# nanoporetech/tombo

Hardware: AMD Instinct MI355X
Metric: resquiggle reads/s (10 kb DNA, bw=500) (higher is better)
Workload: dtype f64

## Files before the change

include/tombo_amd.h:

```cpp
#ifndef TOMBO_AMD_H
#define TOMBO_AMD_H
#include <stdint.h>

#ifdef __cplusplus
extern "C" {
#endif

enum {
    TBA_OK = 0,
    TBA_TOO_MUCH_SIGNAL = 1,
    TBA_FEWER_CPTS = 2,
    TBA_READ_TOO_SHORT_START = 3,
    TBA_MAP_TOO_SHORT_START = 4,
    TBA_POOR_START = 5,
    TBA_INVALID_START_PATH = 6,
    TBA_OPEN_PORE = 7,
    TBA_STARTS_TOO_FAR = 8,
    TBA_MASK_TOO_FEW = 9,
    TBA_ADAPT_BEYOND = 10,
    TBA_BEYOND_BANDWIDTH = 11,
    TBA_DISCORDANT = 12,
    TBA_NOT_ENOUGH_DEL_SIGNAL = 13,
    TBA_TOO_MANY_DELS = 14,
    TBA_INVALID_SEG = 15,
// ... 101 lines not shown
enum {
    TBA_GET_VALID_CPTS = 1,
    TBA_GET_N_CPTS = 2,
    TBA_GET_EVENT_MEANS = 3,
    TBA_GET_SEG_NORM = 4,
    TBA_GET_SEG_SV = 5,
    TBA_GET_START = 6,
    TBA_GET_BAND_STARTS = 7,
    TBA_GET_READ_TB = 8,
    TBA_GET_DP_SEGS = 9,
    TBA_GET_THEIL_SEN = 10,
    TBA_GET_PATH = 11,
    TBA_GET_LAST_ROW = 12,
    TBA_GET_DP_READ_START = 13,
    TBA_GET_KERNEL_MS = 14,
    TBA_GET_REF_MEANS = 15,
    TBA_GET_REF_SDS = 16,
    TBA_GET_SEGS = 17,
    TBA_GET_STATUS = 18,
    TBA_GET_START_FAIL = 19,
    TBA_GET_STALL_INTS = 20,
    TBA_GET_N_STALL = 21,
    TBA_GET_STALL_OFF = 22,
    TBA_GET_SAMP_IND = 23,
    TBA_GET_TB_PARALLEL = 24,
    TBA_GET_ED_FUSED = 25,
    TBA_GET_ED_TAKEN_POS = 26,
    TBA_GET_ED_N_TAKEN = 27,
    TBA_GET_DP_WORKGROUP = 28,
    TBA_GET_ED_FORM = 29,
    TBA_GET_TB_FORM = 30,
    TBA_GET_TB_VERIFY_FAIL = 31,
    TBA_GET_DP_FORM = 32,
    TBA_GET_DEBUG_COUNTERS = 99
};
enum {
    TBA_ED_FORM_NONE = 0,
    TBA_ED_FORM_WG_SCAN_PEAKS = 1,
    TBA_ED_FORM_DETECT_PICK = 2,
    TBA_ED_FORM_SCORES_PEAKS = 3,
    TBA_ED_FORM_DETECT_TT_PICK = 4,
    TBA_ED_FORM_TTEST_PEAKS = 5
};
enum {
    TBA_TB_FORM_NONE = 0,
    TBA_TB_FORM_LANE = 1,
    TBA_TB_FORM_LONG = 2,
    TBA_TB_FORM_PAR16 = 16,
    TBA_TB_FORM_PAR64 = 64
};
enum {
    TBA_DP_FORM_NONE = 0,
    TBA_DP_FORM_K_DP = 1,
    TBA_DP_FORM_K_DP8_LOWREG = 2,
    TBA_DP_FORM_MULTI = 3,
    TBA_DP_FORM_WIDE = 4
};
enum {
    TBA_DP_START_NONE = 0,
    TBA_DP_START_FIRST_TRY = 1,
    TBA_DP_START_RETRY_WG = 2,
    TBA_DP_START_RETRY_K_DP = 3
};
int tba_batch_get(tba_engine *e, int what, void *out, int64_t out_bytes);
enum {
    TBA_STAGE_SEGMENT = 0,
    TBA_STAGE_EVENT_MEANS = 1,
    TBA_STAGE_REF_LEVELS = 2,
    TBA_STAGE_START = 3,
    TBA_STAGE_ASSIGN = 4,
    TBA_STAGE_SKIP = 5,
    TBA_STAGE_RESCALE = 6
};
enum {
    TBA_PUT_VALID_CPTS = 1,
// ... 206 lines not shown
```

tombo_amd/_native.py:

```python
import os
import ctypes as C
import subprocess
from collections import namedtuple

import numpy as np

from ._default_parameters import MAX_POINTS_FOR_THEIL_SEN, SIG_MATCH_THRESH

_HERE = os.path.dirname(os.path.abspath(__file__))
LIB_PATH = os.environ.get('TBA_LIB_PATH') or os.path.join(_HERE, 'libtombo_amd.so')
CSRC = os.path.join(_HERE, 'csrc')
i64, f64, i32 = C.c_int64, C.c_double, C.c_int32

HIPCC_FLAGS = ['--offload-arch=gfx950', '-O3', '-std=c++17', '-ffp-contract=off', '-fPIC',
               '-shared']


INJECT_LIB_PATH = os.path.join(_HERE, 'libtombo_amd_inject.so')
INJECT_FLAGS = ['-DTBA_TB_INJECT=5']


def build(force=False):
    tree_lib = os.path.join(_HERE, 'libtombo_amd.so')
    srcs = [os.path.join(CSRC, f) for f in sorted(os.listdir(CSRC))] + \
# ... 35 lines not shown
                ('device_subsample', i64), ('subsample_seed', C.c_uint64), ('subsample_first_read', i64),
                ('del_fix_window', i64), ('max_del_fix_window', i64), ('extra_sig_factor', f64)]


class ReadResult(C.Structure):
    _fields_ = [('status', i32), ('norm_params_changed', i32),
                ('read_start_rel_to_raw', i64), ('norm_len', i64),
                ('shift', f64), ('scale', f64), ('lower_lim', f64), ('upper_lim', f64),
                ('sig_match_score', f64)]


class SynthParams(C.Structure):
    _fields_ = [('mean_dwell', i64), ('min_dwell', i64), ('n_lead', i64), ('n_trail', i64),
                ('scale', f64), ('offset', f64), ('noise_sd', f64), ('dac_per_pa', f64), ('dac_offset', f64),
                ('reverse', i32), ('pad', i32)]


RESULT_DTYPE = np.dtype([
    ('status', np.int32), ('norm_params_changed', np.int32),
    ('read_start_rel_to_raw', np.int64), ('norm_len', np.int64),
    ('shift', np.float64), ('scale', np.float64), ('lower_lim', np.float64),
    ('upper_lim', np.float64), ('sig_match_score', np.float64)])
assert RESULT_DTYPE.itemsize == C.sizeof(ReadResult) == 64

RAW_F64, RAW_F32, RAW_I16 = 0, 1, 2
RAW_DTYPES = {np.dtype(np.float64): RAW_F64, np.dtype(np.float32): RAW_F32,
              np.dtype(np.int16): RAW_I16}


GET_VALID_CPTS, GET_N_CPTS, GET_EVENT_MEANS, GET_SEG_NORM, GET_SEG_SV, GET_START, \
    GET_BAND_STARTS, GET_READ_TB, GET_DP_SEGS, GET_THEIL_SEN, GET_PATH, GET_LAST_ROW, \
    GET_DP_READ_START, GET_KERNEL_MS, GET_REF_MEANS, GET_REF_SDS, GET_SEGS, GET_STATUS, GET_START_FAIL, \
    GET_STALL_INTS, GET_N_STALL, GET_STALL_OFF, GET_SAMP_IND, GET_TB_PARALLEL, GET_ED_FUSED, GET_ED_TAKEN_POS, GET_ED_N_TAKEN, \
    GET_DP_WORKGROUP, GET_ED_FORM, GET_TB_FORM, GET_TB_VERIFY_FAIL, GET_DP_FORM = range(1, 33)
ED_FORM_NONE, ED_FORM_WG_SCAN_PEAKS, ED_FORM_DETECT_PICK, ED_FORM_SCORES_PEAKS, ED_FORM_DETECT_TT_PICK, \
    ED_FORM_TTEST_PEAKS = range(6)
TB_FORM_NONE, TB_FORM_LANE, TB_FORM_LONG, TB_FORM_PAR16, TB_FORM_PAR64 = 0, 1, 2, 16, 64
DP_FORM_NONE, DP_FORM_K_DP, DP_FORM_K_DP8_LOWREG, DP_FORM_MULTI, DP_FORM_WIDE = range(5)
DP_START_NONE, DP_START_FIRST_TRY, DP_START_RETRY_WG, DP_START_RETRY_K_DP = range(4)
GET_DEBUG_COUNTERS = 99
STAGE_SEGMENT, STAGE_EVENT_MEANS, STAGE_REF_LEVELS, STAGE_START, STAGE_ASSIGN, STAGE_SKIP, \
    STAGE_RESCALE = range(7)
PUT_VALID_CPTS, PUT_EVENT_MEANS, PUT_NORM, PUT_REF_MEANS, PUT_REF_SDS, PUT_DP_SEGS, \
    PUT_START_STATE = range(1, 8)
MAX_BAND = 3072
ABI_VERSION = 12
STAGE_NAMES = ["normalize", "cumsum", "scores", "peaks", "event_means", "ref_levels",
               "start_dp", "start_tb", "prep", "main_dp", "main_tb", "skip_resolve", "theil_sen",
               "rescale_score", "stalls", "total"]

_GET_SHAPES = {
    GET_N_CPTS: (np.int64, ('n',)), GET_DP_READ_START: (np.int64, ('n',)),
    GET_SEG_SV: (np.float64, ('n', 4)), GET_START: (np.float64, ('n', 4)),
    GET_THEIL_SEN: (np.float64, ('n', 4)), GET_PATH: (np.int32, ('n', 4)), GET_DP_FORM: (np.int32, ('n', 4)),
    GET_LAST_ROW: (np.float64, ('n', MAX_BAND)), GET_KERNEL_MS: (np.float32, (32,)),
    GET_DEBUG_COUNTERS: (np.int64, ('n', 8)),
    GET_VALID_CPTS: (np.int64, ('ev',)), GET_EVENT_MEANS: (np.float64, ('ev',)),
    GET_SEG_NORM: (np.float64, ('raw',)),
    GET_BAND_STARTS: (np.int64, ('ref',)), GET_REF_MEANS: (np.float64, ('ref',)), GET_REF_SDS: (np.float64, ('ref',)),
    GET_READ_TB: (np.int64, ('seg',)), GET_DP_SEGS: (np.int64, ('seg',)), GET_SEGS: (np.int64, ('seg',)),
    GET_STATUS: (np.int32, ('n',)), GET_START_FAIL: (np.int32, ('n',)),
    GET_N_STALL: (np.int64, ('n',)), GET_STALL_OFF: (np.int64, ('n',)),
    GET_SAMP_IND: (np.int64, ('n', MAX_POINTS_FOR_THEIL_SEN)),
    GET_TB_PARALLEL: (np.int32, ('n',)), GET_ED_FUSED: (np.int32, ('n',)), GET_DP_WORKGROUP: (np.int32, ('n',)),
    GET_ED_FORM: (np.int32, ('n',)), GET_TB_FORM: (np.int32, ('n',)), GET_TB_VERIFY_FAIL: (np.int32, ('n',)),
    GET_ED_TAKEN_POS: (np.int32, ('raw_x2',)), GET_ED_N_TAKEN: (np.int64, ('n',)),
}

class _Ptr(object):
    _CTYPES = (C.c_int.__mro__[-2], type(C.byref(C.c_int())))

    def __init__(self, dtype, const):
        self.dtype, self.const = np.dtype(dtype), const

    def from_param(self, a):
        if a is None or isinstance(a, self._CTYPES):
            return a
        if isinstance(a, np.ndarray):
            if a.dtype == self.dtype and a.flags.c_contiguous and (self.const or a.flags.writeable):
                return C.c_void_p(a.ctypes.data)
        elif isinstance(a, DeviceArray) and a.dtype == self.dtype:
            return C.c_void_p(a.ptr)
        raise TypeError('expected None, a C-contiguous %s%s array or a ctypes object, got %s' % (
            '' if self.const else 'writeable ', self.dtype, getattr(a, 'dtype', type(a).__name__)))


def _prototypes():
    n, q, u, d, v = C.c_int, i64, C.c_uint64, f64, C.c_void_p
    D, Q, I, B = (_Ptr(t, False) for t in (np.float64, np.int64, np.int32, np.uint8))
    cD, cQ, cI, cB, cS = (_Ptr(t, True) for t in (np.float64, np.int64, np.int32, np.uint8, np.int8))
    P, O, R, SP = (C.POINTER(t) for t in (Params, Opts, ReadResult, SynthParams))
    pileup = [q, cQ, cQ, cS, cQ, q, cQ, cS]
    site_outs = [D, Q, Q, Q, D, Q, Q]
    fwd_pass = [v, D, Q, q, q, Q, cD, q, cD, cD, d, d, d, q, d, n, d]
    return {
        'tba_engine_create': (n, [n, v]),
        'tba_engine_destroy': (None, [v]),
        'tba_last_error': (C.c_char_p, []),
# ... 1369 lines not shown
```

tombo_amd/csrc/k_segment.h:

```cpp
#pragma once
#include "k_select.h"

template <class RT> struct raw_is_int { static constexpr bool value = false; };
template <> struct raw_is_int<int16_t> { static constexpr bool value = true; };
#define NORM_WINDOW_MIN 16384

template <class RT>
__global__ __launch_bounds__(SEL_NT, 4) void k_normalize(ReadState *rs, const DevParams *dp,
    const RT *raw, double *norm, const double *sv_in, int mode, int write_norm)
{
    __shared__ BucketSmem sm;
    ReadState &r = rs[blockIdx.x];
    if (r.status != TBA_OK) return;
    const int tid = threadIdx.x;
    const StampClock<phase_on(PH_NORMALIZE)> stamps(r.dbg);
    const i64 n = r.n_raw;
    const RawSamples<RT> x{raw + r.raw_off};
    double *y = norm + r.raw_off;
    const tba_opts &o = dp->o;
    double shift, scale, lo = 0, hi = 0;
    double xlo = 0, xhi = 0, mn = 0, mx = 0;
    bool have_lims = false, have_dev = false;
    double dlo = 0, dhi = 0;
    if (r.sv_flags & 1) {
        shift = sv_in[4 * blockIdx.x + 0];
        scale = sv_in[4 * blockIdx.x + 1];
        if (r.sv_flags & 2) { have_lims = true; lo = sv_in[4 * blockIdx.x + 2]; hi = sv_in[4 * blockIdx.x + 3]; }
    } else if (mode == 1 && !o.has_const_scale && o.use_rna_event_scale) {
        shift = r.shift; scale = r.scale; have_lims = true; lo = r.lower; hi = r.upper;
    } else {
        double samp[WS_PER];
        double smn = INFINITY, smx = -INFINITY;
#pragma unroll
        for (int q = 0; q < WS_PER; q++) {
            const i64 si = (n * (i64)(q * SEL_NT + tid)) / (SEL_NT * WS_PER);
            samp[q] = x[si];
            smn = samp[q] < smn ? samp[q] : smn; smx = samp[q] > smx ? samp[q] : smx;
        }
        for (int mm = 32; mm >= 1; mm >>= 1) {
            double a = shfl_xor_f64(smn, mm), b2 = shfl_xor_f64(smx, mm);
            smn = a < smn ? a : smn; smx = b2 > smx ? b2 : smx;
        }
        if ((tid & 63) == 0) { sm.redd[2 * (tid >> 6)] = smn; sm.redd[2 * (tid >> 6) + 1] = smx; }
        __syncthreads();
        smn = sm.redd[0]; smx = sm.redd[1];
        for (int w = 1; w < SEL_NT / 64; w++) {
            smn = sm.redd[2 * w] < smn ? sm.redd[2 * w] : smn;
            smx = sm.redd[2 * w + 1] > smx ? sm.redd[2 * w + 1] : smx;
        }
        __syncthreads();
        double span = smx - smn;
        span = span > 0 ? span : 1.0;
        mn = smn - span; mx = smx + span;
        stamps.stamp(0);
        bool have_med = false;
        if constexpr (raw_is_int<RT>::value) {
            if (n >= 4096 && block_int_medians(x, n, (int)smn, (int)smx, &sm, &xlo, &xhi, &dlo, &dhi)) {
                shift = (n & 1) ? xlo : (xlo + xhi) / 2.0;
                have_med = true;
                if (!o.has_const_scale) { scale = (n & 1) ? dlo : (dlo + dhi) / 2.0; have_dev = true; }
            }
            __syncthreads();
        }
        const bool thresh = o.has_outlier_thresh && !(mode == 1 && !o.has_const_scale);
        double med = 0, mad = 0;
#pragma nounroll
        for (int what = 0; what < 3; what++) {
            if (what == 0 && have_med) continue;
            if (what == 1) {
                if (o.has_const_scale) { scale = o.const_scale; continue; }
                if (have_dev) continue;
            }
            if (what == 2) {
                if (!thresh) break;
                const double ylo = (xlo - shift) / scale, yhi = (xhi - shift) / scale;
                med = (n & 1) ? ylo : (ylo + yhi) / 2.0;
                if (have_dev && med == 0.0 && scale > 0) {
                    const double m_lo = dlo / scale, m_hi = dhi / scale;
                    mad = (n & 1) ? m_lo : (m_lo + m_hi) / 2.0;
                    break;
                }
            }
            auto of = [&](double xv) {
                return what == 0 ? xv : (what == 1 ? fabs(xv - shift) : fabs((xv - shift) / scale - med));
            };
            auto val = [&](i64 i) { return of(x[i]); };
            double a_lo = 0, a_hi = 0, res = 0;
            bool done = false;
            if (!raw_is_int<RT>::value && n >= NORM_WINDOW_MIN) {
                double ds[WS_PER];
#pragma unroll
                for (int q = 0; q < WS_PER; q++) ds[q] = of(samp[q]);
                done = block_median_window<2>(x, of, n, ds, y, n, &sm, &a_lo, &a_hi);
                if (done) res = (n & 1) ? a_lo : (a_lo + a_hi) / 2.0;
                __syncthreads();
            }
// ... 771 lines not shown
```

tombo_amd/csrc/k_select.h:

```cpp
#pragma once
#include "tba_common.h"

template <int U, class Load, class Body>
__device__ __forceinline__ void block_stream(i64 n, Load load, Body body)
{
    const i64 tid = threadIdx.x, nt = blockDim.x;
    i64 base = 0;
    for (; base + (i64)U * nt <= n; base += (i64)U * nt) {
        decltype(load((i64)0)) v[U];
#pragma unroll
        for (int u = 0; u < U; u++) v[u] = load(base + (i64)u * nt + tid);
#pragma unroll
        for (int u = 0; u < U; u++) body(base + (i64)u * nt + tid, v[u]);
    }
    for (i64 i = base + tid; i < n; i += nt) body(i, load(i));
}

template <int U, class Sig, class Body>
__device__ __forceinline__ void block_stream2(i64 n, Sig x, Body body)
{
    const i64 tid = threadIdx.x, nt = blockDim.x, np = n >> 1;
    i64 base = 0;
    for (; base + (i64)U * nt <= np; base += (i64)U * nt) {
        double a[U], b[U];
// ... 655 lines not shown
            const i64 a = (shift2 - e) / 2 - base, b2 = (shift2 + e) / 2 - base;
            i64 cnt = 0;
            if (a >= 0 && a < BS_NB) cnt += sm->hist[a];
            if (e != 0 && b2 >= 0 && b2 < BS_NB) cnt += sm->hist[b2];
            c += cnt; loc[q] = c;
        }
        i64 inc = c;
        for (int d = 1; d < 64; d <<= 1) {
            i64 t = shfl_i64(inc, (tid & 63) - d < 0 ? 0 : (tid & 63) - d);
            if ((tid & 63) >= d) inc += t;
        }
        __syncthreads();
        if ((tid & 63) == 63) sm->rad.red[tid >> 6] = (u64)inc;
        __syncthreads();
        i64 off = 0;
        for (int w = 0; w < (tid >> 6); w++) off += (i64)sm->rad.red[w];
        const i64 exc = off + inc - c;
        i64 tot = 0;
        for (int w = 0; w < SEL_NT / 64; w++) tot += (i64)sm->rad.red[w];
        if (tid == 0) s_okk = (tot == n - below - above) && k_hi < tot;
#pragma unroll
        for (int q = 0; q < per; q++) {
            const i64 lo_c = exc + (q ? loc[q - 1] : 0), hi_c = exc + loc[q];
            const i64 e = par + 2 * (i64)(tid * per + q);
            if (lo_c <= k_lo && k_lo < hi_c) s_k[2] = e;
            if (lo_c <= k_hi && k_hi < hi_c) s_k[3] = e;
        }
    }
    __syncthreads();
    if (!s_okk) return false;
    if (below > 0 && (shift2 - s_k[3]) / 2 < (i64)base) return false;
    if (above > 0 && (shift2 + s_k[3]) / 2 > (i64)base + BS_NB - 1) return false;
    *dlo = (double)s_k[2] / 2.0; *dhi = (double)s_k[3] / 2.0;
    return true;
}


__device__ __forceinline__ double seq_sum_lds(const double *p, int j0, int j1, double s = 0)
{
    int j = j0;
    for (; j + 8 <= j1; j += 8) {
        double t[8];
#pragma unroll
        for (int u = 0; u < 8; u++) t[u] = p[j + u];
#pragma unroll
        for (int u = 0; u < 8; u++) s += t[u];
    }
    for (; j < j1; j++) s += p[j];
    return s;
}

template <int SEGW_CAP, class Sig, class F, class Pre, class Emit>
__device__ __forceinline__ void wave_segment_sums(Sig x,
    const i64 *__restrict__ seg, i64 n_segs, i64 first_group, i64 group_stride, double *lds,
    double *out, F f, Pre pre, Emit emit, double mean_len)
{
    constexpr int NP = (SEGW_CAP + 127) / 128;
    const int lane = threadIdx.x & 63;
    int gs = 64;
    while (gs > 4 && (double)gs * mean_len * 1.3 > (double)SEGW_CAP) gs >>= 1;
    i64 g = first_group;
    if (g * gs >= n_segs) return;
    struct Raw { i64 a, hi; };
    auto load_raw = [&](i64 gg) {
        const i64 i = gg * gs + lane;
        const bool ok = lane < gs && i < n_segs;
// ... 165 lines not shown
```

tombo_amd/csrc/tba_common.h:

```cpp
#pragma once
#include <hip/hip_runtime.h>
#include <stdint.h>
#include "../../include/tombo_amd.h"

typedef int64_t i64;
typedef uint64_t u64;
typedef int32_t i32;
typedef uint32_t u32;

#define MASK_BASES 50
#define MASK_FILL_Z_SCORE (-15.0)
#define DEL_FIX_WINDOW 2
#define MAX_DEL_FIX_WINDOW 10
#define EXTRA_SIG_FACTOR 1.1
#define SHIFT_CHANGE_THRESH 0.1
#define SCALE_CHANGE_THRESH 0.1
#define MAX_TS_POINTS 1000

#include "tba_phase.h"

enum { PATH_NONE = 0, PATH_ADAPTIVE = 1, PATH_STATIC = 2 };
enum { ST_NONE = 0, ST_TRY = 1, ST_OK = 2, ST_RETRY = 3, ST_STATIC = 4 };

struct ReadState {
    i64 raw_off, n_raw;
    i64 seq_off, seq_len;
    i64 ref_off, B;
    i64 seg_off;
    i64 ev_off, num_events;
    i64 stall_off, n_stall;
    i32 status, path, start_state, sv_flags;
    i32 n_start_calls, changed, pad0;
    i32 is_long;
    double shift, scale, lower, upper;
    i32 has_lims;
    i32 tb_done;
    i32 ed_flag, dp_wg;
    i32 ed_form, tb_form;
    i32 strip_s0;
    i32 bad_seq;
    i32 tb_verify_fail, pad1;
    i64 n_taken;
    double ed_min, ed_max;
    i64 n_cpts, n_ev;
    double start_res[4];
    i64 mapped_start; double epb;
    i64 clip, offset, W, n_static, moves_off, top_pos;
    i64 read_start, norm_len, dp_read_start;
    i64 n_win, skip_off;
    double ts[4]; double score;
    i64 dbg[8];
};

struct DevParams {
    tba_params p;
    tba_opts o;
    i64 kmer_width, central_pos;
    double fill_masked;
    i32 dp_wg_mode, pad;
};

typedef double f64x2_u __attribute__((ext_vector_type(2), aligned(8)));
typedef float f32x2_u __attribute__((ext_vector_type(2), aligned(4)));
typedef short i16x2_u __attribute__((ext_vector_type(2), aligned(2)));
__device__ __forceinline__ void ld2(const double *p, double &a, double &b)
{
    const f64x2_u v = *(const f64x2_u *)p;
    a = v.x; b = v.y;
}
__device__ __forceinline__ void st2(double *p, double a, double b)
{
    f64x2_u v;
    v.x = a; v.y = b;
    *(f64x2_u *)p = v;
// ... 221 lines not shown
```

tombo_amd/csrc/tba_engine.hip:

```cpp
#include <atomic>
#include "tba_common.h"
#include "k_select.h"
#include "k_segment.h"
#include "k_detect.h"
#include "k_prep_raw.h"
#include "k_dp.h"
#include "k_tb_par.h"
#include "k_dp_multi.h"
#include "k_long.h"
#include "k_dp_wg.h"
#include "k_tail.h"
#include "k_cabi.h"
#include "k_synth.h"
#include "k_group.h"
#include "k_site.h"
#include "k_kde.h"
#include "k_tracks.h"
#include "k_kmer_est.h"
#include "k_roc.h"
#include "k_pdist.h"
#include "k_plot.h"

#include <algorithm>
#include <array>
// ... 542 lines not shown
    c.side = !side_off && first == TBA_STAGE_SEGMENT && last == TBA_STAGE_RESCALE && e->side_mode != 0 &&
             (e->side_mode == 1 || (e->device < TBA_MAX_DEVICES &&
              std::max(e->n_sharing, g_live_engines[e->device].load()) <= max_engines));
    e->last_side = c.side;
    if (c.side && !e->stream2) HIP_TRY(hipStreamCreate(&e->stream2));
    const hipStream_t s2 = c.s2 = c.side ? e->stream2 : s;
    if (c.side) {
        HIP_TRY(hipEventRecord(e->ev_fork, s));
        HIP_TRY(hipStreamWaitEvent(s2, e->ev_fork, 0));
    }
    HIP_TRY(hipEventRecord(e->ev_st0, s2));
    if (first == TBA_STAGE_SEGMENT && c.O.detect_stalls) {
        const unsigned gq = c.gx(e->z.max_raw / 8 + 1);
        if (c.rdt == TBA_RAW_I16 && c.O.stall_window_size <= SI_MAXW) {
            (c.O.stall_n_windows == 7 ? k_stall_metric_i16<7> : k_stall_metric_i16<0>)<<<dim3(gq, c.nb), 256, 0, s2>>>(c.rs, c.dp, (int16_t *)c.raw, c.stall_bits);
        } else {
            if (cs_reads_for(c.n) == 20) RAW_DISPATCH(c.rdt, (k_cumsum_scores<20, RT, 1><<<(unsigned)((c.n + 19) / 20), 256, 0, s2>>>(c.rs, c.n, c.dp, (RT *)c.raw, c.stall_csum)));
            else RAW_DISPATCH(c.rdt, (k_cumsum_scores<32, RT, 1><<<(unsigned)((c.n + 31) / 32), 256, 0, s2>>>(c.rs, c.n, c.dp, (RT *)c.raw, c.stall_csum)));
            if (e->n_long > 0) RAW_DISPATCH(c.rdt, (k_cumsum_scores_long<RT, 1><<<(unsigned)e->n_long, 256, 0, s2>>>(c.rs, c.lng, c.dp, (RT *)c.raw, c.stall_csum)));
            (c.O.stall_n_windows == 7 ? k_stall_metric<7> : k_stall_metric<0>)<<<dim3(gq, c.nb), 256, 0, s2>>>(c.rs, c.dp, c.stall_csum, c.stall_bits);
        }
        k_stall_runs<<<dim3(c.gx(e->z.max_raw / 64 + 1), c.nb), 256, 0, s2>>>(c.rs, c.dp, c.stall_bits, c.stall);
        k_stall_merge<<<c.tpr, 64, 0, s2>>>(c.rs, c.n, c.dp, c.stall);
    }
    HIP_TRY(hipEventRecord(e->ev_st1, s2));
    if (c.side) {
        HIP_TRY(hipEventRecord(e->ev_stalls, s2));
        k_ref_levels<<<dim3(c.gB, c.nb), 256, 0, s2>>>(c.rs, c.dp, c.seq, c.kmeans, c.ksds, c.refm, c.refs, 1);
        HIP_TRY(hipEventRecord(e->ev_levels, s2));
    }
    return 0;
}

static int step_normalize(Run &c)
{
    if (!c.rna) RAW_DISPATCH(c.rdt, (k_normalize<RT><<<c.nb, SEL_NT, 0, c.s>>>(c.rs, c.dp, (RT *)c.raw, c.norm, c.sv_in, 0, c.fused_detect && !c.wg_scan ? 2 : 1)));
    return 0;
}
static int step_cumsum(Run &c)
{
    const i64 n = c.n;
    if (c.rna) return 0;
    if (c.wg_scan) {
        k_cumsum_scores_long<double, 0><<<c.nb, 256, 0, c.s>>>(c.rs, c.order, c.dp, c.norm, c.score);
        return 0;
    }
    if (c.fused_detect) {
        RAW_DISPATCH(c.rdt, (k_detect<2, RT><<<(unsigned)((n + DT_READS - 1) / DT_READS), 256, 0, c.s>>>(c.rs, n, c.dp, (RT *)c.raw, c.norm, c.csum, c.score, c.e->z.S_tot)));
        k_pick<<<c.nb, SEL_NT, 0, c.s>>>(c.rs, c.dp, c.csum, c.score, c.cpts, 0);
    }
    if (c.fused_scores) {
        if (cs_reads_for(n) == 20) k_cumsum_scores<20><<<(unsigned)((n + 19) / 20), 256, 0, c.s>>>(c.rs, n, c.dp, c.norm, c.score, c.only_flagged);
        else k_cumsum_scores<32><<<(unsigned)((n + 31) / 32), 256, 0, c.s>>>(c.rs, n, c.dp, c.norm, c.score, c.only_flagged);
        if (c.e->n_long > 0) k_cumsum_scores_long<double, 0><<<(unsigned)c.e->n_long, 256, 0, c.s>>>(c.rs, c.lng, c.dp, c.norm, c.score);
    }
    else k_cumsum<<<c.tpr, 64, 0, c.s>>>(c.rs, n, c.norm, c.csum);
    return 0;
}
static int step_scores(Run &c)
{
    if (!c.rna) {
        if (!c.fused_scores) k_scores_dna<<<dim3(c.gS, c.nb), 256, 0, c.s>>>(c.rs, c.dp, c.csum, c.score);
        return 0;
    }
    if (c.fused_tt) {
        if (c.P.running_stat_width == 12) RAW_DISPATCH(c.rdt, (k_detect_tt<5, 12, RT><<<c.nb, SEL_NT, 0, c.s>>>(c.rs, c.dp, (RT *)c.raw, c.csum, c.score)));
        else RAW_DISPATCH(c.rdt, (k_detect_tt<5, 0, RT><<<c.nb, SEL_NT, 0, c.s>>>(c.rs, c.dp, (RT *)c.raw, c.csum, c.score)));
        k_pick<<<c.nb, SEL_NT, 0, c.s>>>(c.rs, c.dp, c.csum, c.score, c.cpts, 1);
    }
    RAW_DISPATCH(c.rdt, (k_scores_ttest<RT><<<dim3(c.gS, c.nb), 256, 0, c.s>>>(c.rs, c.dp, (RT *)c.raw, c.score, c.only_flagged)));
    return 0;
}
static int step_peaks(Run &c)
{
    launch_peaks(c.P.min_obs_per_base, c.nb, c.s, c.rs, c.dp, c.score, c.state, c.csum, c.cpts, c.rna ? 1 : 0, c.only_flagged,
                 c.rna ? TBA_ED_FORM_TTEST_PEAKS : c.wg_scan ? TBA_ED_FORM_WG_SCAN_PEAKS : TBA_ED_FORM_SCORES_PEAKS);
    if (c.side) HIP_TRY(hipStreamWaitEvent(c.s, c.e->ev_stalls, 0));
    if (c.e->any_stall) k_remove_stalls<<<c.nb, SEL_NT, 0, c.s>>>(c.rs, c.n, c.stall, c.cpts, c.csum);
    if (c.rna) {
        RAW_DISPATCH(c.rdt, (k_event_means<RT, 1280><<<dim3(c.gE, c.nb), 256, 0, c.s>>>(c.rs, c.dp, (RT *)c.raw, c.cpts, c.evm, 1)));
        k_rna_event_scale<<<c.nb, SEL_NT, 0, c.s>>>(c.rs, c.dp, c.evm);
        RAW_DISPATCH(c.rdt, (k_normalize<RT><<<c.nb, SEL_NT, 0, c.s>>>(c.rs, c.dp, (RT *)c.raw, c.norm, c.sv_in, 1, 1)));
    }
    return 0;
}
static int step_event_means(Run &c)
{
    (c.P.mean_obs_per_event >= 10 ? k_event_means<double, 1280> : k_event_means<double>)<<<dim3(c.gE, c.nb), 256, 0, c.s>>>(c.rs, c.dp, c.norm, c.cpts, c.evm, 0);
    return 0;
}
static int step_ref_levels(Run &c)
{
    if (c.side) {
        HIP_TRY(hipStreamWaitEvent(c.s, c.e->ev_levels, 0));
        k_seq_status<<<c.tpr, 64, 0, c.s>>>(c.rs, c.n);
    } else
        k_ref_levels<<<dim3(c.gB, c.nb), 256, 0, c.s>>>(c.rs, c.dp, c.seq, c.kmeans, c.ksds, c.refm, c.refs);
    return 0;
}
static void launch_start_tb(Run &c, int mode)
{
    k_start_tb<<<(unsigned)((c.n + TB_LANES - 1) / TB_LANES), TB_LANES, 0, c.s>>>(c.rs, c.n, c.dp, mode, c.evm, c.refm, c.refs, c.smoves, c.e->z.start_moves_stride, c.readtb, c.startvals);
}
static int step_start_dp(Run &c)
{
    k_path0<<<c.tpr, 64, 0, c.s>>>(c.rs, c.n, c.dp);
    launch_dp(c, cpl_class(c.P.start_bw), DP_START_TRY);
    launch_start_tb(c, DP_START_TRY);
    return 0;
}
static int step_start_tb(Run &c)
{
    const int wcpl = c.P.start_n_bases <= WG_MAX_ROWS ? dp_wg_cpl(c.P.start_save_bw) : 0;
    c.e->last_dp.start = true, c.e->last_dp.retry_wcpl = wcpl;
    const auto wg = wcpl == 4 ? k_dp_wg<4> : wcpl == 8 ? k_dp_wg<8> : wcpl == 12 ? k_dp_wg<12> : nullptr;
// ... 332 lines not shown
    case TBA_GET_SEGS: return copy(e->d_segs, e->n_segs() * 8);
    case TBA_GET_SAMP_IND: return copy(e->d_samp, N * MAX_TS_POINTS * 8);
    case TBA_GET_STALL_INTS:
        if (!e->any_stall) return set_err(TBA_E_STATE, "the batch has no stall intervals");
        return copy(e->d_stall, std::min((size_t)e->z.n_stall * 16, (size_t)out_bytes));
    case TBA_GET_KERNEL_MS:
        if ((size_t)out_bytes < sizeof(e->stage_ms)) return set_err(TBA_E_ARG, "output buffer too small");
        memcpy(out, e->stage_ms, sizeof(e->stage_ms));
        return 0;
    default: break;
    }
    std::vector<ReadState> rs(N);
    HIP_TRY(hipMemcpy(rs.data(), e->d_rs.p, N * sizeof(ReadState), hipMemcpyDeviceToHost));
    auto per_read = [&](auto get) -> int {
        typedef decltype(get(rs[0])) T;
        if ((size_t)out_bytes < N * sizeof(T)) return set_err(TBA_E_ARG, "output buffer too small");
        for (size_t i = 0; i < N; i++) {
            const T v = get(rs[i]);
            memcpy((char *)out + i * sizeof(T), &v, sizeof(T));
        }
        return 0;
    };
#define PER_READ(T, ...) per_read([](const ReadState &r) -> T { return __VA_ARGS__; })
    typedef std::array<double, 4> D4;
    typedef std::array<i32, 4> I4;
    typedef std::array<i64, 8> I8;
    switch (what) {
    case TBA_GET_START_FAIL: return PER_READ(i32, r.pad0);
    case TBA_GET_STATUS: return PER_READ(i32, r.status);
    case TBA_GET_ED_FUSED: return PER_READ(i32, r.ed_form == TBA_ED_FORM_DETECT_PICK || r.ed_form == TBA_ED_FORM_DETECT_TT_PICK);
    case TBA_GET_TB_PARALLEL: return PER_READ(i32, r.tb_done);
    case TBA_GET_ED_FORM: return PER_READ(i32, r.ed_form);
    case TBA_GET_TB_FORM: return PER_READ(i32, r.tb_form);
    case TBA_GET_TB_VERIFY_FAIL: return PER_READ(i32, r.tb_verify_fail);
    case TBA_GET_DP_WORKGROUP: return PER_READ(i32, r.dp_wg);
    case TBA_GET_ED_N_TAKEN: return PER_READ(i64, r.n_taken);
    case TBA_GET_N_CPTS: return PER_READ(i64, r.n_cpts);
    case TBA_GET_DP_READ_START: return PER_READ(i64, r.dp_read_start);
    case TBA_GET_N_STALL: return PER_READ(i64, r.n_stall);
    case TBA_GET_STALL_OFF: return PER_READ(i64, r.stall_off);
    case TBA_GET_SEG_SV: return PER_READ(D4, D4{r.shift, r.scale, r.lower, r.upper});
    case TBA_GET_START: return PER_READ(D4, to_array(r.start_res));
    case TBA_GET_THEIL_SEN: return PER_READ(D4, to_array(r.ts));
    case TBA_GET_PATH: return PER_READ(I4, I4{r.path, (i32)r.n_static, (i32)r.W, r.n_start_calls});
    case TBA_GET_DEBUG_COUNTERS: return PER_READ(I8, to_array(r.dbg));
    case TBA_GET_DP_FORM: {
        const tba_params &P = e->hp.p;
        const tba_engine::DpLaunches L = e->last_dp;
        const int multi_cpl = dp_multi_class(P.bandwidth).cpl;
        const int retry_cpl = L.retry_wcpl ? L.retry_wcpl : cpl_class(P.start_save_bw);
        return per_read([&](const ReadState &r) -> I4 {
            I4 f{TBA_DP_FORM_NONE, 0, TBA_DP_START_NONE, 0};
            if (L.main && r.path != PATH_NONE) {
                const int c = cpl_class(r.W);
                if (r.path == PATH_ADAPTIVE && r.W == P.bandwidth && multi_cpl != 0)
                    f[0] = TBA_DP_FORM_MULTI, f[1] = multi_cpl;
                else if (c != 0)
                    f[0] = c == 8 && L.lowreg ? TBA_DP_FORM_K_DP8_LOWREG : TBA_DP_FORM_K_DP, f[1] = c;
                else if (r.path == PATH_STATIC && L.wide)
                    f[0] = TBA_DP_FORM_WIDE;
            }
            const bool retried = r.n_start_calls == 2 || r.start_state == ST_RETRY;
            const bool tried = retried || r.n_start_calls == 1 || r.pad0 != 0 || r.start_state == ST_TRY;
            if (L.start && retried)
                f[2] = L.retry_wcpl ? TBA_DP_START_RETRY_WG : TBA_DP_START_RETRY_K_DP, f[3] = retry_cpl;
            else if (L.start && tried)
// ... 2171 lines not shown
```

Measured before the change: 111,700.

## Add histogram-based median/MAD normalization pre-pass for float raw signals

Adds a k_normalize_hist kernel that builds a block-wide histogram of the raw signal, uses prefix sums to locate the median and MAD buckets, and compacts only the candidate samples into a short list. Exact median and MAD are then selected from that list instead of running the full selection over all samples. k_normalize reuses the precomputed shift, scale and limits when the histogram path succeeds and falls back to the existing selection otherwise. This costs an extra kernel launch and full passes over the raw data per read, and it is skipped for int16 raw input.

```diff
diff --git a/include/tombo_amd.h b/include/tombo_amd.h
--- a/include/tombo_amd.h
+++ b/include/tombo_amd.h
@@ -157,6 +157,7 @@
     TBA_GET_TB_FORM = 30,
     TBA_GET_TB_VERIFY_FAIL = 31,
     TBA_GET_DP_FORM = 32,
+    TBA_GET_NORM_FORM = 33,
     TBA_GET_DEBUG_COUNTERS = 99
 };
 enum {
@@ -166,6 +167,12 @@
     TBA_ED_FORM_SCORES_PEAKS = 3,
     TBA_ED_FORM_DETECT_TT_PICK = 4,
     TBA_ED_FORM_TTEST_PEAKS = 5
+};
+enum {
+    TBA_NORM_FORM_NONE = 0,
+    TBA_NORM_FORM_SELECT = 1,
+    TBA_NORM_FORM_INT_COUNT = 2,
+    TBA_NORM_FORM_HIST = 3
 };
 enum {
     TBA_TB_FORM_NONE = 0,
diff --git a/tombo_amd/_native.py b/tombo_amd/_native.py
--- a/tombo_amd/_native.py
+++ b/tombo_amd/_native.py
@@ -91,9 +91,10 @@
     GET_BAND_STARTS, GET_READ_TB, GET_DP_SEGS, GET_THEIL_SEN, GET_PATH, GET_LAST_ROW, \
     GET_DP_READ_START, GET_KERNEL_MS, GET_REF_MEANS, GET_REF_SDS, GET_SEGS, GET_STATUS, GET_START_FAIL, \
     GET_STALL_INTS, GET_N_STALL, GET_STALL_OFF, GET_SAMP_IND, GET_TB_PARALLEL, GET_ED_FUSED, GET_ED_TAKEN_POS, GET_ED_N_TAKEN, \
-    GET_DP_WORKGROUP, GET_ED_FORM, GET_TB_FORM, GET_TB_VERIFY_FAIL, GET_DP_FORM = range(1, 33)
+    GET_DP_WORKGROUP, GET_ED_FORM, GET_TB_FORM, GET_TB_VERIFY_FAIL, GET_DP_FORM, GET_NORM_FORM = range(1, 34)
 ED_FORM_NONE, ED_FORM_WG_SCAN_PEAKS, ED_FORM_DETECT_PICK, ED_FORM_SCORES_PEAKS, ED_FORM_DETECT_TT_PICK, \
     ED_FORM_TTEST_PEAKS = range(6)
+NORM_FORM_NONE, NORM_FORM_SELECT, NORM_FORM_INT_COUNT, NORM_FORM_HIST = range(4)
 TB_FORM_NONE, TB_FORM_LANE, TB_FORM_LONG, TB_FORM_PAR16, TB_FORM_PAR64 = 0, 1, 2, 16, 64
 DP_FORM_NONE, DP_FORM_K_DP, DP_FORM_K_DP8_LOWREG, DP_FORM_MULTI, DP_FORM_WIDE = range(5)
 DP_START_NONE, DP_START_FIRST_TRY, DP_START_RETRY_WG, DP_START_RETRY_K_DP = range(4)
@@ -122,7 +123,7 @@
     GET_N_STALL: (np.int64, ('n',)), GET_STALL_OFF: (np.int64, ('n',)),
     GET_SAMP_IND: (np.int64, ('n', MAX_POINTS_FOR_THEIL_SEN)),
     GET_TB_PARALLEL: (np.int32, ('n',)), GET_ED_FUSED: (np.int32, ('n',)), GET_DP_WORKGROUP: (np.int32, ('n',)),
-    GET_ED_FORM: (np.int32, ('n',)), GET_TB_FORM: (np.int32, ('n',)), GET_TB_VERIFY_FAIL: (np.int32, ('n',)),
+    GET_NORM_FORM: (np.int32, ('n',)), GET_ED_FORM: (np.int32, ('n',)), GET_TB_FORM: (np.int32, ('n',)), GET_TB_VERIFY_FAIL: (np.int32, ('n',)),
     GET_ED_TAKEN_POS: (np.int32, ('raw_x2',)), GET_ED_N_TAKEN: (np.int64, ('n',)),
 }
 
diff --git a/tombo_amd/csrc/k_segment.h b/tombo_amd/csrc/k_segment.h
--- a/tombo_amd/csrc/k_segment.h
+++ b/tombo_amd/csrc/k_segment.h
@@ -4,6 +4,65 @@
 template <class RT> struct raw_is_int { static constexpr bool value = false; };
 template <> struct raw_is_int<int16_t> { static constexpr bool value = true; };
 #define NORM_WINDOW_MIN 16384
+
+__host__ __device__ __forceinline__ bool batch_has_medians(const tba_opts &o, int mode)
+{
+    return !o.has_const_scale && !(mode == 1 && o.use_rna_event_scale);
+}
+__device__ __forceinline__ bool norm_needs_medians(const ReadState &r, const tba_opts &o, int mode)
+{
+    return !(r.sv_flags & 1) && !(mode == 1 && !o.has_const_scale && o.use_rna_event_scale);
+}
+template <class X>
+__device__ __forceinline__ void norm_sample_range(X x, i64 n, BucketSmem *sm, double *smn_out, double *smx_out)
+{
+    const int tid = threadIdx.x;
+    double smn = INFINITY, smx = -INFINITY;
+#pragma unroll
+    for (int q = 0; q < WS_PER; q++) {
+        const i64 si = (n * (i64)(q * SEL_NT + tid)) / (SEL_NT * WS_PER);
+        const double v = x[si];
+        smn = v < smn ? v : smn; smx = v > smx ? v : smx;
+    }
+    for (int mm = 32; mm >= 1; mm >>= 1) {
+        double a = shfl_xor_f64(smn, mm), b2 = shfl_xor_f64(smx, mm);
+        smn = a < smn ? a : smn; smx = b2 > smx ? b2 : smx;
+    }
+    if ((tid & 63) == 0) { sm->redd[2 * (tid >> 6)] = smn; sm->redd[2 * (tid >> 6) + 1] = smx; }
+    __syncthreads();
+    smn = sm->redd[0]; smx = sm->redd[1];
+    for (int w = 1; w < SEL_NT / 64; w++) {
+        smn = sm->redd[2 * w] < smn ? sm->redd[2 * w] : smn;
+        smx = sm->redd[2 * w + 1] > smx ? sm->redd[2 * w + 1] : smx;
+    }
+    __syncthreads();
+    *smn_out = smn; *smx_out = smx;
+}
+
+template <class RT>
+__global__ __launch_bounds__(SEL_NT, 4) void k_normalize_hist(ReadState *rs, const DevParams *dp,
+    const RT *raw, double *norm, int mode)
+{
+    __shared__ BucketSmem sm;
+    ReadState &r = rs[blockIdx.x];
+    if (r.status != TBA_OK) return;
+    const tba_opts &o = dp->o;
+    const i64 n = r.n_raw;
+    if (!batch_has_medians(o, mode) || !norm_needs_medians(r, o, mode) || n < NORM_WINDOW_MIN) return;
+    const RawSamples<RT> x{raw + r.raw_off};
+    double smn, smx;
+    norm_sample_range(x, n, &sm, &smn, &smx);
+    const bool thresh = o.has_outlier_thresh && mode != 1;
+    HistMedians hm;
+    if (!block_hist_medians(x, n, smn, smx, thresh, norm + r.raw_off, &sm, &hm)) return;
+    if (threadIdx.x == 0) {
+        r.shift = hm.shift; r.scale = hm.scale;
+        r.lower = thresh ? hm.med - (hm.mad * o.outlier_thresh) : 0.0;
+        r.upper = thresh ? hm.med + (hm.mad * o.outlier_thresh) : 0.0;
+        r.has_lims = thresh ? 1 : 0;
+        r.norm_form = TBA_NORM_FORM_HIST;
+    }
+}
 
 template <class RT>
 __global__ __launch_bounds__(SEL_NT, 4) void k_normalize(ReadState *rs, const DevParams *dp,
@@ -28,6 +87,8 @@
         if (r.sv_flags & 2) { have_lims = true; lo = sv_in[4 * blockIdx.x + 2]; hi = sv_in[4 * blockIdx.x + 3]; }
     } else if (mode == 1 && !o.has_const_scale && o.use_rna_event_scale) {
         shift = r.shift; scale = r.scale; have_lims = true; lo = r.lower; hi = r.upper;
+    } else if (r.norm_form == TBA_NORM_FORM_HIST) {
+        shift = r.shift; scale = r.scale; have_lims = r.has_lims != 0; lo = r.lower; hi = r.upper;
     } else {
         double samp[WS_PER];
         double smn = INFINITY, smx = -INFINITY;
@@ -62,6 +123,7 @@
             }
             __syncthreads();
         }
+        if (tid == 0) r.norm_form = have_med ? TBA_NORM_FORM_INT_COUNT : TBA_NORM_FORM_SELECT;
         const bool thresh = o.has_outlier_thresh && !(mode == 1 && !o.has_const_scale);
         double med = 0, mad = 0;
 #pragma nounroll
diff --git a/tombo_amd/csrc/k_select.h b/tombo_amd/csrc/k_select.h
--- a/tombo_amd/csrc/k_select.h
+++ b/tombo_amd/csrc/k_select.h
@@ -711,6 +711,221 @@
     if (below > 0 && (shift2 - s_k[3]) / 2 < (i64)base) return false;
     if (above > 0 && (shift2 + s_k[3]) / 2 > (i64)base + BS_NB - 1) return false;
     *dlo = (double)s_k[2] / 2.0; *dhi = (double)s_k[3] / 2.0;
+    return true;
+}
+
+#define NH_CAP 4096
+struct HistMedians { double shift, scale, med, mad; };
+struct NhPlan {
+    int bl, bh, la, lb, ra, rb, ok;
+    i64 c_below, c_inner, c_outl, c_outr, n_brk, n_list;
+};
+__device__ __forceinline__ bool nh_in(int b, int lo, int hi) { return (u32)(b - lo) <= (u32)(hi - lo); }
+
+template <class F>
+__device__ __forceinline__ void nh_two_kth(F val, i64 m, i64 k_lo, i64 k_hi, double lo, double hi, BucketSmem *sm,
+                                           double *a_out, double *b_out)
+{
+    const double a = block_kth(val, m, k_lo, lo, hi, sm);
+    const int found = sm->found;
+    const double nxt = sm->next;
+    __syncthreads();
+    double b = a;
+    if (k_hi != k_lo) {
+        if (found & 2) b = nxt;
+        else { b = block_kth(val, m, k_hi, lo, hi, sm); __syncthreads(); }
+    }
+    *a_out = a; *b_out = b;
+}
+
+template <class X>
+__device__ bool block_hist_medians(X x, i64 n, double smn, double smx, bool want_mad, double *list,
+                                   BucketSmem *sm, HistMedians *out)
+{
+    const int tid = threadIdx.x, lane = tid & 63;
+    __shared__ NhPlan s_p;
+    __shared__ int s_b[4];
+    __shared__ u32 s_nl;
+    __shared__ double s_ext[4 * (SEL_NT / 64)];
+    if (!(smx > smn) || n > 0x7fffffff) return false;
+    const double hsc = (double)BS_NB / (smx - smn);
+    if (!(hsc < 1e300) || !(hsc > 0.0)) return false;
+    for (int b = tid; b < BS_NB; b += SEL_NT) sm->hist[b] = 0;
+    if (tid == 0) { s_nl = 0; s_p.ok = 1; }
+    __syncthreads();
+    bool bad = false;
+    block_stream2<4>(n, x, [&](i64, double v) {
+        bad |= v != v;
+        atomicAdd(&sm->hist[bs_bucket(v, smn, hsc)], 1u);
+    });
+    if (bad) s_p.ok = 0;
+    __syncthreads();
+    {
+        constexpr int per = BS_NB / SEL_NT;
+        u32 loc[per], c = 0;
+#pragma unroll
+        for (int q = 0; q < per; q++) { c += sm->hist[tid * per + q]; loc[q] = c; }
+        u32 inc = c;
+        for (int d = 1; d < 64; d <<= 1) {
+            const u32 t = (u32)__shfl_up((int)inc, d, 64);
+            if (lane >= d) inc += t;
+        }
+        if (lane == 63) sm->rad.red[tid >> 6] = inc;
+        __syncthreads();
+        u32 off = 0;
+        for (int w = 0; w < (tid >> 6); w++) off += (u32)sm->rad.red[w];
+        const u32 exc = off + inc - c;
+#pragma unroll
+        for (int q = 0; q < per; q++) sm->hist[tid * per + q] = exc + loc[q];
+    }
+    __syncthreads();
+    auto P = [&](int b) -> i64 { return b < 0 ? 0 : (i64)sm->hist[b < BS_NB - 1 ? b : BS_NB - 1]; };
+    const i64 k_lo = (n - 1) / 2, k_hi = n / 2;
+    for (int b = tid; b < BS_NB; b += SEL_NT) {
+        const i64 lo_c = P(b - 1), hi_c = P(b);
+        if (lo_c <= k_lo && k_lo < hi_c) s_b[0] = b;
+        if (lo_c <= k_hi && k_hi < hi_c) s_b[1] = b;
+    }
+    __syncthreads();
+    {
+        const int bl = s_b[0], bh = s_b[1];
+        for (int s = tid; s < BS_NB; s += SEL_NT) {
+            const i64 u = P(bh + s) - P(bl - s - 1), up = s ? P(bh + s - 1) - P(bl - s) : 0;
+            if (up < k_lo + 1 && u >= k_lo + 1) s_b[2] = s;
+            if (up < k_hi + 1 && u >= k_hi + 1) s_b[3] = s;
+        }
+    }
+    __syncthreads();
+    if (tid == 0) {
+        const int bl = s_b[0], bh = s_b[1], s1 = s_b[2], s1p = s_b[3];
+        int la = bl - s1p - 1, rb = bh + s1p + 1;
+        const int lb = bh - s1 + 1, ra = bl + s1 - 1;
+        bool ok = s_p.ok && bh - bl <= 1 && lb < bl && ra > bh && lb >= 0 && ra <= BS_NB - 1;
+        la = la > 0 ? la : 0; rb = rb < BS_NB - 1 ? rb : BS_NB - 1;
+        if (ok) {
+            const i64 n_l = P(lb) - P(la - 1), n_m = P(bh) - P(bl - 1), n_r = P(rb) - P(ra - 1);
+            ok = n_l > 0 && n_r > 0 && n_l + n_m + n_r <= NH_CAP;
+            s_p.bl = bl; s_p.bh = bh; s_p.la = la; s_p.lb = lb; s_p.ra = ra; s_p.rb = rb;
+            s_p.c_below = P(bl - 1); s_p.c_inner = P(ra - 1) - P(lb);
+            s_p.c_outl = P(la - 1); s_p.c_outr = n - P(rb);
+            s_p.n_brk = n_l + n_r; s_p.n_list = n_l + n_m + n_r;
+        }
+        s_p.ok = ok;
+    }
+    __syncthreads();
+    if (!s_p.ok) return false;
+    const int bl = s_p.bl, bh = s_p.bh, la = s_p.la, lb = s_p.lb, ra = s_p.ra, rb = s_p.rb;
+    const i64 m = s_p.n_list;
+    {
+        constexpr int WU = 4;
+        const i64 np = (n + 1) >> 1;
+        for (i64 base = 0; base < np; base += (i64)WU * SEL_NT) {
+            double v[2 * WU];
+            bool okv[2 * WU];
+#pragma unroll
+            for (int u = 0; u < WU; u++) {
+                const i64 i = 2 * (base + (i64)u * SEL_NT + tid);
+                okv[2 * u] = i < n; okv[2 * u + 1] = i + 1 < n;
+                if (i + 1 < n) sig_pair(x, i, v[2 * u], v[2 * u + 1]);
+                else { v[2 * u] = x[i < n ? i : n - 1]; v[2 * u + 1] = v[2 * u]; }
+            }
+            u64 mk[2 * WU];
+            u32 tot = 0;
+#pragma unroll
+            for (int u = 0; u < 2 * WU; u++) {
+                const int b = bs_bucket(v[u], smn, hsc);
+                mk[u] = __ballot(okv[u] && (nh_in(b, la, lb) || nh_in(b, bl, bh) || nh_in(b, ra, rb)));
+                tot += (u32)__popcll(mk[u]);
+            }
+            if (tot) {
+                u32 b0 = 0;
+                if (lane == 0) b0 = atomicAdd(&s_nl, tot);
+                b0 = __shfl(b0, 0, 64);
+#pragma unroll
+                for (int u = 0; u < 2 * WU; u++) {
+                    const u32 pos = b0 + (u32)__popcll(mk[u] & ((1ull << lane) - 1ull));
+                    if (((mk[u] >> lane) & 1ull) && pos < NH_CAP) list[pos] = v[u];
+                    b0 += (u32)__popcll(mk[u]);
+                }
+            }
+        }
+    }
+    __threadfence_block();
+    __syncthreads();
+    if ((i64)s_nl != m) return false;
+    {
+        double o_l = INFINITY, m_l = -INFINITY, m_r = INFINITY, o_r = -INFINITY;
+        for (i64 i = tid; i < m; i += SEL_NT) {
+            const double v = list[i];
+            const int b = bs_bucket(v, smn, hsc);
+            if (nh_in(b, la, lb)) { o_l = v < o_l ? v : o_l; m_l = v > m_l ? v : m_l; }
+            else if (nh_in(b, ra, rb)) { m_r = v < m_r ? v : m_r; o_r = v > o_r ? v : o_r; }
+        }
+        for (int mm = 32; mm >= 1; mm >>= 1) {
+            const double a = shfl_xor_f64(o_l, mm), b2 = shfl_xor_f64(m_l, mm), c2 = shfl_xor_f64(m_r, mm),
+                         d2 = shfl_xor_f64(o_r, mm);
+            o_l = a < o_l ? a : o_l; m_l = b2 > m_l ? b2 : m_l; m_r = c2 < m_r ? c2 : m_r; o_r = d2 > o_r ? d2 : o_r;
+        }
+        if (lane == 0) {
+            double *e = s_ext + 4 * (tid >> 6);
+            e[0] = o_l; e[1] = m_l; e[2] = m_r; e[3] = o_r;
+        }
+    }
+    __syncthreads();
+    if (tid == 0) {
+        double o_l = s_ext[0], m_l = s_ext[1], m_r = s_ext[2], o_r = s_ext[3];
+        for (int w = 1; w < SEL_NT / 64; w++) {
+            const double *e = s_ext + 4 * w;
+            o_l = e[0] < o_l ? e[0] : o_l; m_l = e[1] > m_l ? e[1] : m_l;
+            m_r = e[2] < m_r ? e[2] : m_r; o_r = e[3] > o_r ? e[3] : o_r;
+        }
+        s_ext[0] = o_l; s_ext[1] = m_l; s_ext[2] = m_r; s_ext[3] = o_r;
+    }
+    if (k_lo - s_p.c_inner < 0 || k_hi - s_p.c_inner >= s_p.n_brk) return false;
+    __syncthreads();
+    double xlo = 0, xhi = 0, shift = 0, dlo = 0, dhi = 0, scale = 1, med = 0, mad = 0;
+#pragma nounroll
+    for (int what = 0; what < 3; what++) {
+        if (what == 2) {
+            if (!want_mad) break;
+            const double ylo = (xlo - shift) / scale, yhi = (xhi - shift) / scale;
+            med = (n & 1) ? ylo : (ylo + yhi) / 2.0;
+            if (med == 0.0) {
+                const double m_lo = dlo / scale, m_hi = dhi / scale;
+                mad = (n & 1) ? m_lo : (m_lo + m_hi) / 2.0;
+                break;
+            }
+        }
+        auto g = [&](double v) { return what == 1 ? v - shift : (v - shift) / scale - med; };
+        auto val = [&](i64 i) {
+            const double v = list[i];
+            const int b = bs_bucket(v, smn, hsc);
+            if (what == 0) return nh_in(b, bl, bh) ? v : INFINITY;
+            return nh_in(b, la, lb) || nh_in(b, ra, rb) ? fabs(g(v)) : INFINITY;
+        };
+        const i64 c_off = what == 0 ? s_p.c_below : s_p.c_inner;
+        const double w_lo = (double)(s_b[2] > 2 ? s_b[2] - 2 : 0) / hsc, w_hi = (double)(s_b[3] + 3) / hsc;
+        const double r_lo = what == 0 ? smn + (double)bl / hsc : (what == 1 ? w_lo : w_lo / scale);
+        const double r_hi = what == 0 ? smn + (double)(bh + 1) / hsc : (what == 1 ? w_hi : w_hi / scale);
+        double a_lo, a_hi;
+        nh_two_kth(val, m, k_lo - c_off, k_hi - c_off, r_lo, r_hi, sm, &a_lo, &a_hi);
+        if (what == 0) {
+            xlo = a_lo; xhi = a_hi;
+            shift = (n & 1) ? xlo : (xlo + xhi) / 2.0;
+            continue;
+        }
+        const double g_l = g(s_ext[1]), g_r = g(s_ext[2]);
+        bool ok = g_l <= 0.0 && g_r >= 0.0 && fabs(g_l) <= a_lo && fabs(g_r) <= a_lo;
+        if (s_p.c_outl > 0) ok = ok && fabs(g(s_ext[0])) >= a_hi;
+        if (s_p.c_outr > 0) ok = ok && fabs(g(s_ext[3])) >= a_hi;
+        if (!ok) return false;
+        const double res = (n & 1) ? a_lo : (a_lo + a_hi) / 2.0;
+        if (what == 1) {
+            dlo = a_lo; dhi = a_hi; scale = res;
+            if (!(scale > 0.0)) return false;
+        } else mad = res;
+    }
+    out->shift = shift; out->scale = scale; out->med = med; out->mad = mad;
     return true;
 }
 
diff --git a/tombo_amd/csrc/tba_common.h b/tombo_amd/csrc/tba_common.h
--- a/tombo_amd/csrc/tba_common.h
+++ b/tombo_amd/csrc/tba_common.h
@@ -39,7 +39,8 @@
     i32 ed_form, tb_form;
     i32 strip_s0;
     i32 bad_seq;
-    i32 tb_verify_fail, pad1;
+    i32 tb_verify_fail;
+    i32 norm_form;
     i64 n_taken;
     double ed_min, ed_max;
     i64 n_cpts, n_ev;
diff --git a/tombo_amd/csrc/tba_engine.hip b/tombo_amd/csrc/tba_engine.hip
--- a/tombo_amd/csrc/tba_engine.hip
+++ b/tombo_amd/csrc/tba_engine.hip
@@ -598,9 +598,18 @@
     return 0;
 }
 
+static void launch_normalize(Run &c, int mode, int write_norm)
+{
+    if (batch_has_medians(c.O, mode)) {
+        if (c.rdt == TBA_RAW_F32) k_normalize_hist<float><<<c.nb, SEL_NT, 0, c.s>>>(c.rs, c.dp, (float *)c.raw, c.norm, mode);
+        else if (c.rdt != TBA_RAW_I16) k_normalize_hist<double><<<c.nb, SEL_NT, 0, c.s>>>(c.rs, c.dp, (double *)c.raw, c.norm, mode);
+    }
+    RAW_DISPATCH(c.rdt, (k_normalize<RT><<<c.nb, SEL_NT, 0, c.s>>>(c.rs, c.dp, (RT *)c.raw, c.norm, c.sv_in, mode, write_norm)));
+}
+
 static int step_normalize(Run &c)
 {
-    if (!c.rna) RAW_DISPATCH(c.rdt, (k_normalize<RT><<<c.nb, SEL_NT, 0, c.s>>>(c.rs, c.dp, (RT *)c.raw, c.norm, c.sv_in, 0, c.fused_detect && !c.wg_scan ? 2 : 1)));
+    if (!c.rna) launch_normalize(c, 0, c.fused_detect && !c.wg_scan ? 2 : 1);
     return 0;
 }
 static int step_cumsum(Run &c)
@@ -646,7 +655,7 @@
     if (c.rna) {
         RAW_DISPATCH(c.rdt, (k_event_means<RT, 1280><<<dim3(c.gE, c.nb), 256, 0, c.s>>>(c.rs, c.dp, (RT *)c.raw, c.cpts, c.evm, 1)));
         k_rna_event_scale<<<c.nb, SEL_NT, 0, c.s>>>(c.rs, c.dp, c.evm);
-        RAW_DISPATCH(c.rdt, (k_normalize<RT><<<c.nb, SEL_NT, 0, c.s>>>(c.rs, c.dp, (RT *)c.raw, c.norm, c.sv_in, 1, 1)));
+        launch_normalize(c, 1, 1);
     }
     return 0;
 }
@@ -1045,6 +1054,7 @@
     case TBA_GET_TB_PARALLEL: return PER_READ(i32, r.tb_done);
     case TBA_GET_ED_FORM: return PER_READ(i32, r.ed_form);
     case TBA_GET_TB_FORM: return PER_READ(i32, r.tb_form);
+    case TBA_GET_NORM_FORM: return PER_READ(i32, r.norm_form);
     case TBA_GET_TB_VERIFY_FAIL: return PER_READ(i32, r.tb_verify_fail);
     case TBA_GET_DP_WORKGROUP: return PER_READ(i32, r.dp_wg);
     case TBA_GET_ED_N_TAKEN: return PER_READ(i64, r.n_taken);
```

Result: faster. 114,600, median of 6 (+2.6%).
